# pavel-paulau/query

Hardware: AMD Instinct MI355X
Metric: rows/sec filter+group-by on 100M synthetic JSON docs; achieved HBM GB/s (higher is better)
Workload: dtype int64/f64 tagged scalars (u8 tag + 8 B payload), u32 dictionary codes; 1 GPU; config2: SELECT cat, SUM(price) FROM default WHERE price > 50 GROUP BY cat @ 100000000 rows, K_cat=1000, columns resident in HBM; rows_per_gpu=100000000, groups=1000, rows_selected=49401294, agg_mode=2, spec_kernel=1

## Files before the change

### query_amd/csrc/n1k_kernels.hip

```cpp
#include <hip/hip_runtime.h>
#include "n1k_device.h"
#include "n1k_tables.h"
#include "n1k_scatter.h"
#include "n1k_kernels.h"
#include <algorithm>
#include <vector>

namespace n1k {


template <int R>
N1K_DEV void load_operand(const Program& P, const Operand& o, const uint64_t (&row)[R], const bool (&valid)[R],
                          uint32_t (&tag)[R], uint64_t (&pay)[R]) {
    if (o.is_const) {
#pragma unroll
        for (int j = 0; j < R; j++) {
            tag[j] = o.ctag;
            pay[j] = o.cpayload;
        }
        return;
    }
    const DevCol& c = P.cols[o.col];
    if (c.kind == COLK_DICT32) {
        const uint32_t* codes = c.codes;
// ... 1185 lines not shown
                    unpackable = 1;
                    pass[j] = false;
                }
                key[j] = mix64(key[j] ^ canon) + k;
            }
        }
        uint64_t pos[R];
        uint32_t dest[R];
#pragma unroll
        for (int j = 0; j < R; j++) {
            dest[j] = (uint32_t)(((key[j] >> 32) * (uint64_t)A.nparts) >> 32);
            pos[j] = 0;
            for (uint32_t d = 0; d < A.nparts; d++) {
                unsigned long long m = __ballot(pass[j] && dest[j] == d);
                if (m == 0ull) continue;
                int leader = __ffsll((long long)m) - 1;
                uint32_t base = 0;
                if ((int)lane == leader) base = atomicAdd(&s_cnt[d], (uint32_t)__popcll(m));
                base = __shfl(base, leader, 64);
                if (pass[j] && dest[j] == d) pos[j] = base + (uint32_t)__popcll(m & ((1ull << lane) - 1ull));
            }
        }
        __syncthreads();
        for (uint32_t d = tid; d < A.nparts; d += BLOCK) {
            uint32_t n = s_cnt[d];
            s_base[d] = n ? atomicAdd(&A.counts[(size_t)d * (A.count_stride ? A.count_stride : 1u)], (unsigned long long)n) : 0ull;
        }
        __syncthreads();
#pragma unroll
        for (int j = 0; j < R; j++) {
            if (!pass[j]) continue;
            uint64_t r = s_base[dest[j]] + pos[j];
            if (r >= (A.per_dest ? (uint64_t)A.dest_cap[dest[j]] : A.capacity)) {
                if (!(atomicOr(A.err_flags, (uint32_t)ERR_TABLE_FULL) & ERR_TABLE_FULL) && A.region_bytes)
                    for (uint32_t q = 0; q < A.nparts; q++)
                        atomicOr(&A.counts[(size_t)q * A.count_stride + 1], 1ull);
                pass[j] = false;
            }
            pos[j] = A.region_bytes ? r : (uint64_t)dest[j] * A.capacity + r;
        }
        __syncthreads();
        for (uint32_t d = tid; d < A.nparts; d += BLOCK) s_cnt[d] = 0;
        uint64_t roff[R];
#pragma unroll
        for (int j = 0; j < R; j++) roff[j] = A.hdr_bytes;
        for (uint32_t c = 0; c < A.ncopy; c++) {
            Operand o{};
            o.is_const = 0;
            o.col = c;
            uint32_t vt[R];
            uint64_t vp[R];
            load_operand<R>(P, o, row, pass, vt, vp);
#pragma unroll
            for (int j = 0; j < R; j++) {
                if (!pass[j]) continue;
                if (A.per_dest) {
                    char* const reg = (char*)A.counts + (size_t)dest[j] * A.region_bytes;
                    const uint64_t capd = A.dest_cap[dest[j]];
                    if (P.cols[c].kind == COLK_DICT32) {
                        ((uint32_t*)(reg + roff[j]))[pos[j]] = (uint32_t)vp[j];
                        roff[j] = part_region_next(roff[j], capd, 4);
                    } else {
                        ((uint64_t*)(reg + roff[j]))[pos[j]] = vp[j];
                        roff[j] = part_region_next(roff[j], capd, 8);
                        ((uint8_t*)(reg + roff[j]))[pos[j]] = (uint8_t)vt[j];
                        roff[j] = part_region_next(roff[j], capd, 1);
                    }
                    continue;
                }
                const size_t shift = (size_t)dest[j] * A.region_bytes;
                if (P.cols[c].kind == COLK_DICT32) {
                    ((uint32_t*)((char*)A.out_codes[c] + shift))[pos[j]] = (uint32_t)vp[j];
                } else {
                    ((uint8_t*)((char*)A.out_tags[c] + shift))[pos[j]] = (uint8_t)vt[j];
                    ((uint64_t*)((char*)A.out_payload[c] + shift))[pos[j]] = vp[j];
                }
            }
        }
    }
    if (unsupported) atomicOr(A.err_flags, (uint32_t)ERR_UNSUPPORTED_VALUE);
    if (unpackable) atomicOr(A.err_flags, (uint32_t)ERR_UNPACKABLE_KEY);
}

enum { RED_ADD_U64, RED_ADD_F64, RED_OR, RED_MIN_I64, RED_MAX_I64, RED_MIN_U64, RED_MAX_U64 };

template <int OP>
N1K_DEV uint64_t reduce_over_y(uint64_t (*red)[64], uint64_t v) {
    const uint32_t tx = threadIdx.x, ty = threadIdx.y;
    red[ty][tx] = v;
    __syncthreads();
    for (uint32_t off = 8; off > 0; off >>= 1) {
        if (ty < off) {
            uint64_t a = red[ty][tx], b = red[ty + off][tx], r;
            if (OP == RED_ADD_U64) r = a + b;
            else if (OP == RED_ADD_F64) r = f64_bits(as_f64(a) + as_f64(b));
            else if (OP == RED_OR) r = a | b;
            else if (OP == RED_MIN_I64) r = (int64_t)a < (int64_t)b ? a : b;
            else if (OP == RED_MAX_I64) r = (int64_t)a > (int64_t)b ? a : b;
            else if (OP == RED_MIN_U64) r = a < b ? a : b;
            else r = a > b ? a : b;
            red[ty][tx] = r;
        }
        __syncthreads();
    }
    uint64_t out = red[0][tx];
    __syncthreads();
    return out;
}

__global__ __launch_bounds__(1024) void merge_slabs_kernel(const Program P, const FastArgs F, const GlobalTable G,
                                                          uint32_t nblocks_total, unsigned long long* ngroups) {
    __shared__ uint64_t red[16][64];
    const uint32_t S = F.lds_slots;
    const uint32_t s = blockIdx.x * 64 + threadIdx.x;
    const bool in_range = s < S;
    if (blockIdx.x == 0 && blockIdx.y == 0 && threadIdx.y == 0) {
        unsigned long long c = 0;
        for (uint32_t b = threadIdx.x; b < nblocks_total; b += 64) c += F.block_selected[b];
        for (int off = 32; off > 0; off >>= 1) c += __shfl_down(c, off, 64);
        if (threadIdx.x == 0 && c) atomicAdd(F.rows_selected, c);
    }
    const uint32_t Y = 16 * gridDim.y, y = blockIdx.y * 16 + threadIdx.y;
    const size_t slab_words = (size_t)P.lds_words * S * Y;
    const uint32_t nblocks = (in_range && y < nblocks_total) ? (nblocks_total - y + Y - 1) / Y : 0;
    const uint64_t* base = F.slabs + (size_t)y * P.lds_words * S + (in_range ? s : 0);
    uint64_t touched = 0;
#pragma unroll 8
    for (uint32_t b = 0; b < nblocks; b++) touched |= base[b * slab_words] ^ kEmptyKey;
    touched = reduce_over_y<RED_OR>(red, touched);
    const bool leader = threadIdx.y == 0 && in_range && touched != 0;
    long long g = -1;
    if (leader) g = global_find_or_insert(G, fast_slot_key(F, s), F.err_flags, ngroups);
    uint64_t* grow = g >= 0 ? &G.acc[(size_t)g * P.glob_words] : nullptr;
    for (uint32_t a = 0; a < P.naggs; a++) {
        const AggSpec& ag = P.aggs[a];
        if (ag.distinct) continue;
        const uint64_t* l = base + (size_t)ag.lds_off * S;
        unsigned long long* w = grow ? (unsigned long long*)(grow + ag.glob_off) : nullptr;
        switch (ag.kind) {
            case AGG_COUNT:
            case AGG_COUNTN: {
                unsigned long long c = 0;
#pragma unroll 8
                for (uint32_t b = 0; b < nblocks; b++) c += l[b * slab_words];
                c = reduce_over_y<RED_ADD_U64>(red, c);
                if (w && c) atomicAdd(&w[0], c);
                break;
            }
            case AGG_SUM:
            case AGG_AVG: {
                unsigned long long lo = 0, hi = 0, fl = 0, n = 0;
                double fs = 0.0;
                const bool avg = ag.kind == AGG_AVG;
#pragma unroll 4
                for (uint32_t b = 0; b < nblocks; b++) {
                    const uint64_t* lb = l + b * slab_words;
                    int64_t x = (int64_t)lb[0];
                    double f = as_f64(lb[(size_t)S]);
                    fl |= lb[2 * (size_t)S];
                    lo += (unsigned long long)(uint32_t)x;
                    hi += (unsigned long long)(x >> 32);
                    fs += f;
                    if (avg) n += lb[3 * (size_t)S];
                }
                lo = reduce_over_y<RED_ADD_U64>(red, lo);
                hi = reduce_over_y<RED_ADD_U64>(red, hi);
                fs = as_f64(reduce_over_y<RED_ADD_F64>(red, f64_bits(fs)));
                fl = reduce_over_y<RED_OR>(red, fl);
                if (avg) n = reduce_over_y<RED_ADD_U64>(red, n);
                if (!w || !fl) break;
                if (fl & (SF_NONNEG_INT | SF_NEG_INT)) { atomicAdd(&w[0], lo); atomicAdd(&w[1], hi); }
                if (fl & SF_FLOAT) atomicAdd((double*)&w[2], fs);
                atomicOr(&w[3], fl);
                if (avg) atomicAdd(&w[4], n);
                break;
            }
            default: {
                const bool mn = ag.kind == AGG_MIN;
                unsigned long long fl = 0;
                long long iv = mn ? INT64_MAX : INT64_MIN;
                unsigned long long fv = mn ? ~0ull : 0ull, sv = mn ? ~0ull : 0ull;
#pragma unroll 4
                for (uint32_t b = 0; b < nblocks; b++) {
                    const uint64_t* lb = l + b * slab_words;
                    fl |= lb[0];
                    long long x = (long long)lb[(size_t)S];
                    unsigned long long yv = lb[2 * (size_t)S], z = lb[3 * (size_t)S];
                    iv = mn ? (x < iv ? x : iv) : (x > iv ? x : iv);
                    fv = mn ? (yv < fv ? yv : fv) : (yv > fv ? yv : fv);
                    sv = mn ? (z < sv ? z : sv) : (z > sv ? z : sv);
                }
                fl = reduce_over_y<RED_OR>(red, fl);
                if (mn) {
                    iv = (long long)reduce_over_y<RED_MIN_I64>(red, (uint64_t)iv);
                    fv = reduce_over_y<RED_MIN_U64>(red, fv);
                    sv = reduce_over_y<RED_MIN_U64>(red, sv);
                } else {
                    iv = (long long)reduce_over_y<RED_MAX_I64>(red, (uint64_t)iv);
                    fv = reduce_over_y<RED_MAX_U64>(red, fv);
                    sv = reduce_over_y<RED_MAX_U64>(red, sv);
                }
                if (!w || !fl) break;
                atomicOr(&w[0], fl);
                if (fl & MM_INT) { if (mn) atomicMin((long long*)&w[1], iv); else atomicMax((long long*)&w[1], iv); }
                if (fl & MM_FLOAT) { if (mn) atomicMin(&w[2], fv); else atomicMax(&w[2], fv); }
                if (fl & MM_STRING) { if (mn) atomicMin(&w[3], sv); else atomicMax(&w[3], sv); }
                break;
            }
        }
    }
}

__global__ void export_partials_kernel(const Program P, const GlobalTable G, uint32_t nparts, uint64_t cap,
                                       uint64_t* out, uint64_t region_words, uint32_t* err_flags) {
    uint64_t s = (uint64_t)blockIdx.x * blockDim.x + threadIdx.x;
    if (s == 0 && P.wide_count && *P.wide_count)
        for (uint32_t r = 0; r < nparts; r++) atomicOr((unsigned long long*)&out[(size_t)r * region_words + 1], 2ull);
    const uint64_t key = s < G.capacity ? G.keys[s] : kEmptyKey;
    const bool used = key != kEmptyKey;
    const uint32_t d = used ? (uint32_t)(((mix64(key) >> 32) * (uint64_t)nparts) >> 32) : 0xFFFFFFFFu;
    unsigned long long pos = 0;
    unsigned long long todo = __ballot(used);
    const uint32_t lane = threadIdx.x & 63;
    while (todo) {
        const int leader = __ffsll((long long)todo) - 1;
        const uint32_t dl = __shfl(d, leader, 64);
        const unsigned long long same = __ballot(used && d == dl);
        unsigned long long base = 0;
        if ((int)lane == leader) base = atomicAdd((unsigned long long*)&out[(size_t)dl * region_words], (unsigned long long)__popcll(same));
        base = __shfl(base, leader, 64);
        if (used && d == dl) pos = base + (unsigned long long)__popcll(same & ((1ull << lane) - 1ull));
        todo &= ~same;
    }
    if (!used) return;
    uint64_t* region = out + (size_t)d * region_words;
    if (pos >= cap) {
        if (!(atomicOr(err_flags, (uint32_t)ERR_TABLE_FULL) & ERR_TABLE_FULL))
            for (uint32_t r = 0; r < nparts; r++) atomicOr((unsigned long long*)&out[(size_t)r * region_words + 1], 1ull);
        return;
    }
    region[2 + pos] = key;
    uint64_t* acc = region + 2 + cap + pos * P.glob_words;
    for (uint32_t w = 0; w < P.glob_words; w++) acc[w] = G.acc[(size_t)s * P.glob_words + w];
}

N1K_DEV void merge_partial_record(const Program& P, const GlobalTable& G, uint64_t key, const uint64_t* l, uint32_t* err_flags,
                                  bool& fresh, bool unique_keys) {
    long long g = global_find_or_insert_quiet(G, key, err_flags, fresh);
    if (g < 0) return;
    if (fresh && unique_keys) {
        uint64_t* w = &G.acc[(size_t)g * P.glob_words];
        for (uint32_t i = 0; i < P.glob_words; i++) w[i] = l[i];
        return;
    }
    for (uint32_t a = 0; a < P.naggs; a++) {
        const AggSpec& ag = P.aggs[a];
        const uint64_t* p = l + ag.glob_off;
        unsigned long long* w = (unsigned long long*)&G.acc[(size_t)g * P.glob_words + ag.glob_off];
        if (ag.distinct) {
            atomicOr(err_flags, (uint32_t)ERR_UNSUPPORTED_VALUE);
            continue;
        }
        switch (ag.kind) {
            case AGG_COUNT:
            case AGG_COUNTN:
                if (p[0]) atomicAdd(&w[0], (unsigned long long)p[0]);
                break;
            case AGG_SUM:
            case AGG_AVG:
                if (!p[3]) break;
                atomicAdd(&w[0], (unsigned long long)p[0]);
                atomicAdd(&w[1], (unsigned long long)p[1]);
                if (p[3] & SF_FLOAT) atomicAdd((double*)&w[2], as_f64(p[2]));
                atomicOr(&w[3], (unsigned long long)p[3]);
                if (ag.kind == AGG_AVG) atomicAdd(&w[4], (unsigned long long)p[4]);
                break;
            default: {
                if (!p[0]) break;
                bool mn = ag.kind == AGG_MIN;
                atomicOr(&w[0], (unsigned long long)p[0]);
                if (p[0] & MM_INT) { if (mn) atomicMin((long long*)&w[1], (long long)p[1]); else atomicMax((long long*)&w[1], (long long)p[1]); }
                if (p[0] & MM_FLOAT) { if (mn) atomicMin(&w[2], (unsigned long long)p[2]); else atomicMax(&w[2], (unsigned long long)p[2]); }
                if (p[0] & MM_STRING) { if (mn) atomicMin(&w[3], (unsigned long long)p[3]); else atomicMax(&w[3], (unsigned long long)p[3]); }
                break;
            }
        }
    }
}

N1K_DEV void raise_verdict(uint64_t verdict, uint32_t* err_flags) {
    uint32_t f = 0;
    if (verdict & VD_OVERFLOW) f |= ERR_EXCHANGE_OVERFLOW;
// ... 155 lines not shown
            else which = (fl & MM_OTHER) ? 4 : ((fl & MM_STRING) ? 3 : (has_num ? 2 : (has_bool ? 1 : 0)));
            if (which == 1) {
                tag = mn ? ((fl & MM_FALSE) ? T_FALSE : T_TRUE) : ((fl & MM_TRUE) ? T_TRUE : T_FALSE);
            } else if (which == 2) {
                bool hi = fl & MM_INT, hf = fl & MM_FLOAT;
                double f = f64_unsortable(w[2]);
                int64_t iv = (int64_t)w[1];
                bool pick_int = hi;
                if (hi && hf) {
                    int c = collate_f64((double)iv, f);
                    pick_int = mn ? c <= 0 : c >= 0;
                }
                if (pick_int) { tag = T_INT; p = (uint64_t)iv; }
                else { tag = T_FLOAT; p = f64_bits(f); }
            } else if (which == 3) {
                tag = T_STRING;
                p = w[3] & 0xFFFFFFFFull;
            } else if (which == 4) {
                atomicOr(err_flags, (uint32_t)ERR_UNSUPPORTED_VALUE);
            }
            pt.ext_tag = tag;
            pt.ext_payload = p;
            put_value(fin, tag, p);
            break;
        }
    }
    *part = pt;
}

constexpr uint32_t kFinalizeChunkMax = 16384;
__global__ __launch_bounds__(256) void finalize_kernel(const Program P, const GlobalTable G, OutValue* out_keys, OutValue* out_aggs,
                                                       OutPartial* out_parts, uint64_t* out_rep, unsigned long long* out_count,
                                                       uint64_t max_out, uint32_t* err_flags, uint32_t chunk) {
    __shared__ uint32_t wave_cnt[4];
    __shared__ unsigned long long chunk_base;
    const uint32_t tid = threadIdx.x, lane = tid & 63, wave = tid >> 6;
    const uint64_t lo = (uint64_t)blockIdx.x * chunk;
    const uint64_t hi = lo + chunk < G.capacity ? lo + chunk : G.capacity;
    uint32_t mine = 0;
    for (uint64_t s = lo + tid; s < hi; s += 256) mine += G.keys[s] != kEmptyKey ? 1u : 0u;
    for (int off = 32; off > 0; off >>= 1) mine += __shfl_down(mine, off, 64);
    if (lane == 0) wave_cnt[wave] = mine;
    __syncthreads();
    if (tid == 0) {
        const uint32_t total = wave_cnt[0] + wave_cnt[1] + wave_cnt[2] + wave_cnt[3];
        chunk_base = total ? atomicAdd(out_count, (unsigned long long)total) : 0ull;
    }
    __syncthreads();
    unsigned long long next = chunk_base;
    for (uint64_t s0 = lo; s0 < hi; s0 += 256) {
        const uint64_t s = s0 + tid;
        const uint64_t key = s < hi ? G.keys[s] : kEmptyKey;
        const bool used = key != kEmptyKey;
        const unsigned long long m = __ballot(used);
        __syncthreads();
        if (lane == 0) wave_cnt[wave] = (uint32_t)__popcll(m);
        __syncthreads();
        uint32_t before = 0;
        for (uint32_t w = 0; w < wave; w++) before += wave_cnt[w];
        const uint32_t step_total = wave_cnt[0] + wave_cnt[1] + wave_cnt[2] + wave_cnt[3];
        const unsigned long long idx = next + before + (uint32_t)__popcll(m & ((1ull << lane) - 1ull));
        next += step_total;
        if (!used || idx >= max_out) continue;
        for (uint32_t k = 0; k < P.nkeys; k++) {
            const KeySpec& ks = P.keys[k];
            uint64_t field = ks.bits >= 64 ? key : ((key >> ks.shift) & ((1ull << ks.bits) - 1ull));
            uint32_t tag;
            uint64_t p;
            unpack_key_field(P, ks.mode, field, tag, p);
            put_value(&out_keys[idx * P.nkeys + k], tag, p);
        }
        const uint64_t* g = &G.acc[(size_t)s * P.glob_words];
        for (uint32_t a = 0; a < P.naggs; a++)
            finalize_agg(P, P.aggs[a], g, &out_aggs[idx * P.naggs + a], &out_parts[idx * P.naggs + a], err_flags);
        if (out_rep) out_rep[idx] = P.emit_packed_key ? key : (G.rep_row ? G.rep_row[s] : ~0ull);
    }
}

constexpr uint32_t kFinalizeSmallMax = 8192;
__global__ __launch_bounds__(1024) void finalize_small_kernel(const Program P, const GlobalTable G, OutValue* out_keys, OutValue* out_aggs,
                                                             OutPartial* out_parts, uint64_t* out_rep, unsigned long long* counters,
                                                             unsigned long long* host_counters, uint64_t max_out, uint32_t* err_flags,
                                                             uint32_t clear) {
    __shared__ uint32_t wave_cnt[16];
    const uint32_t tid = threadIdx.x, lane = tid & 63, wave = tid >> 6;
    unsigned long long next = 0;
    for (uint64_t s0 = 0; s0 < G.capacity; s0 += 1024) {
        const uint64_t s = s0 + tid;
        const uint64_t key = s < G.capacity ? G.keys[s] : kEmptyKey;
        const bool used = key != kEmptyKey;
        const unsigned long long m = __ballot(used);
        __syncthreads();
        if (lane == 0) wave_cnt[wave] = (uint32_t)__popcll(m);
        __syncthreads();
        uint32_t before = 0, step_total = 0;
        for (uint32_t w = 0; w < 16; w++) {
            before += w < wave ? wave_cnt[w] : 0u;
            step_total += wave_cnt[w];
        }
        const unsigned long long idx = next + before + (uint32_t)__popcll(m & ((1ull << lane) - 1ull));
        next += step_total;
        if (!used) continue;
        uint64_t* g = &G.acc[(size_t)s * P.glob_words];
        if (idx < max_out) {
            for (uint32_t k = 0; k < P.nkeys; k++) {
                const KeySpec& ks = P.keys[k];
                uint64_t field = ks.bits >= 64 ? key : ((key >> ks.shift) & ((1ull << ks.bits) - 1ull));
                uint32_t tag;
                uint64_t p;
                unpack_key_field(P, ks.mode, field, tag, p);
                put_value(&out_keys[idx * P.nkeys + k], tag, p);
            }
            for (uint32_t a = 0; a < P.naggs; a++)
                finalize_agg(P, P.aggs[a], g, &out_aggs[idx * P.naggs + a], &out_parts[idx * P.naggs + a], err_flags);
            if (out_rep) out_rep[idx] = P.emit_packed_key ? key : (G.rep_row ? G.rep_row[s] : ~0ull);
        }
        if (clear) {
            G.keys[s] = kEmptyKey;
            if (G.rep_row) G.rep_row[s] = ~0ull;
            glob_row_init(P, g);
        }
    }
    __syncthreads();
    if (tid == 0) counters[2] = next;
    __syncthreads();
    if (tid < kCounters) {
        host_counters[tid] = __hip_atomic_load(&counters[tid], __ATOMIC_RELAXED, __HIP_MEMORY_SCOPE_AGENT);
        if (clear) counters[tid] = 0;
    }
}

hipError_t launch_finalize_small(const Program& P, const GlobalTable& G, OutValue* out_keys, OutValue* out_aggs, OutPartial* out_parts,
                                 uint64_t* out_rep, unsigned long long* counters, unsigned long long* host_counters, uint64_t max_out,
                                 uint32_t* err_flags, bool clear, hipStream_t st) {
    if (G.capacity > kFinalizeSmallMax) return hipErrorInvalidValue;
    hipLaunchKernelGGL(finalize_small_kernel, dim3(1), dim3(1024), 0, st, P, G, out_keys, out_aggs, out_parts, out_rep, counters,
                       host_counters, max_out, err_flags, clear ? 1u : 0u);
    return hipGetLastError();
}

N1K_DEV uint64_t order_image(const Program& P, uint64_t tag, uint64_t p, bool desc);
__global__ void finalize_region_kernel(const Program P, const uint64_t* region, uint64_t cap, uint64_t count, OutValue* out_keys,
                                       OutValue* out_aggs, OutPartial* out_parts, uint64_t* out_rep, uint32_t* err_flags,
                                       const uint32_t* cand, OutValue* ord, uint32_t ord_is_key, uint32_t ord_index, uint64_t* images,
                                       uint32_t desc) {
    const uint64_t j = (uint64_t)blockIdx.x * blockDim.x + threadIdx.x;
    if (j >= count) return;
    const uint64_t i = cand ? (uint64_t)cand[j] : j;
    const uint64_t key = region[2 + i];
    const uint64_t* g = region + 2 + cap + i * P.glob_words;
    if (ord || images) {
        OutValue v, term;
        OutPartial part;
        term.tag = T_MISSING;
        term.payload = 0;
        for (uint32_t a = 0; a < P.naggs; a++) {
            finalize_agg(P, P.aggs[a], g, &v, &part, err_flags);
            if (!ord_is_key && a == ord_index) term = v;
        }
        if (ord_is_key) {
            const KeySpec& ks = P.keys[ord_index];
            uint64_t field = ks.bits >= 64 ? key : ((key >> ks.shift) & ((1ull << ks.bits) - 1ull));
            uint32_t tag;
            uint64_t p;
            unpack_key_field(P, ks.mode, field, tag, p);
            put_value(&term, tag, p);
        }
        if (images) images[i] = order_image(P, term.tag, term.payload, desc != 0);
        else ord[i] = term;
        return;
    }
    for (uint32_t k = 0; k < P.nkeys; k++) {
        const KeySpec& ks = P.keys[k];
        uint64_t field = ks.bits >= 64 ? key : ((key >> ks.shift) & ((1ull << ks.bits) - 1ull));
        uint32_t tag;
        uint64_t p;
        unpack_key_field(P, ks.mode, field, tag, p);
        put_value(&out_keys[j * P.nkeys + k], tag, p);
    }
    for (uint32_t a = 0; a < P.naggs; a++)
        finalize_agg(P, P.aggs[a], g, &out_aggs[j * P.naggs + a], &out_parts[j * P.naggs + a], err_flags);
    if (out_rep) out_rep[j] = ~0ull;
}

template <int R, int BLOCK>
__global__ __launch_bounds__(BLOCK) void project_records_kernel(const Program P, const ProjectArgs A) {
    __shared__ uint32_t wave_cnt[BLOCK / 64];
    __shared__ unsigned long long tile_base;
    __shared__ uint32_t s_hist[256];
    const uint32_t tid = threadIdx.x;
    for (uint32_t i = tid; i < 256; i += BLOCK) s_hist[i] = 0;
    __syncthreads();
    uint32_t unsupported = 0, unpackable = 0;
    const uint64_t tile_rows = (uint64_t)BLOCK * R;
    const uint64_t ntiles = (A.nrows + tile_rows - 1) / tile_rows;
    for (uint64_t tile = blockIdx.x; tile < ntiles; tile += gridDim.x) {
        uint64_t row[R];
// ... 750 lines not shown
        } else {
            tag = T_STRING;
            pay = a.k_cat;
        }
        if (a.price_tags) a.price_tags[j] = tag;
        if (a.price_payload) a.price_payload[j] = pay;
    }
    uint64_t urange = a.total_rows / 10;
    if (urange == 0) urange = 1;
    if (a.user_tags) a.user_tags[j] = T_INT;
    if (a.user_payload) a.user_payload[j] = splitmix64(base + 3) % urange;
    if (a.region_tags) a.region_tags[j] = T_INT;
    if (a.region_payload) a.region_payload[j] = splitmix64(base + 4) % 64ull;
}


hipError_t launch_init_table(const Program& P, const GlobalTable& G, uint64_t first, uint64_t count,
                             unsigned long long* counters, hipStream_t st) {
    if (count == 0) return hipSuccess;
    uint32_t blocks = (uint32_t)((count + 255) / 256);
    hipLaunchKernelGGL(init_table_kernel, dim3(blocks), dim3(256), 0, st, P, G, first, count, counters);
    return hipGetLastError();
}

hipError_t launch_rehash(const Program& P, const GlobalTable& oldt, const GlobalTable& newt, uint32_t* err_flags,
                         unsigned long long* ngroups_scratch, hipStream_t st) {
    uint32_t blocks = (uint32_t)((oldt.capacity + 255) / 256);
    hipLaunchKernelGGL(rehash_kernel, dim3(blocks), dim3(256), 0, st, P, oldt, newt, err_flags, ngroups_scratch);
    return hipGetLastError();
}

template <int R, int BLOCK>
static hipError_t launch_scan_variant(const Program& P, const ScanArgs& A, const GlobalTable& G, unsigned long long* ngroups,
                                      uint32_t grid, bool direct, size_t shmem, hipStream_t st) {
    if (direct) {
        auto k = scan_group_kernel<R, BLOCK, true>;
        if (shmem > 48 * 1024) (void)hipFuncSetAttribute((const void*)k, hipFuncAttributeMaxDynamicSharedMemorySize, (int)shmem);
        hipLaunchKernelGGL(k, dim3(grid), dim3(BLOCK), shmem, st, P, A, G, ngroups);
    } else {
        auto k = scan_group_kernel<R, BLOCK, false>;
        if (shmem > 48 * 1024) (void)hipFuncSetAttribute((const void*)k, hipFuncAttributeMaxDynamicSharedMemorySize, (int)shmem);
        hipLaunchKernelGGL(k, dim3(grid), dim3(BLOCK), shmem, st, P, A, G, ngroups);
    }
    return hipGetLastError();
}

hipError_t launch_scan_group(const Program& P, const ScanArgs& A, const GlobalTable& G, unsigned long long* ngroups,
                             uint32_t grid, uint32_t block, uint32_t rows_per_lane, bool direct, hipStream_t st) {
    size_t shmem = (size_t)A.lds_slots * P.lds_words * 8 + (size_t)A.dcache_slots * A.dcache_aggs * 8;
    if (block == 256) return launch_scan_variant<4, 256>(P, A, G, ngroups, grid, direct, shmem, st);
    if (block == 512) return launch_scan_variant<4, 512>(P, A, G, ngroups, grid, direct, shmem, st);
    if (rows_per_lane == 2) return launch_scan_variant<2, 1024>(P, A, G, ngroups, grid, direct, shmem, st);
    return launch_scan_variant<4, 1024>(P, A, G, ngroups, grid, direct, shmem, st);
}

template <int R, int BLOCK>
static hipError_t launch_fast_variant(const Program& P, const FastArgs& F, const GlobalTable& G, unsigned long long* ngroups,
                                      uint32_t grid, size_t shmem, hipStream_t st) {
    auto k = scan_fast_kernel<R, BLOCK>;
    if (shmem > 48 * 1024) (void)hipFuncSetAttribute((const void*)k, hipFuncAttributeMaxDynamicSharedMemorySize, (int)shmem);
    hipLaunchKernelGGL(k, dim3(grid), dim3(BLOCK), shmem, st, P, F, G, ngroups);
    return hipGetLastError();
}

hipError_t launch_scan_fast(const Program& P, const FastArgs& F, const GlobalTable& G, unsigned long long* ngroups,
                            uint32_t grid, uint32_t block, uint32_t rows_per_lane, hipStream_t st) {
    size_t shmem = (size_t)F.lds_slots * P.lds_words * 8;
    for (uint32_t t = 0; t < F.nterms; t++)
        if (term_is_table_bit(F.terms[t].op) && F.terms[t].like_n <= kLikeLdsBytes) {
            shmem += kLikeLdsBytes;
            break;
        }
    if (block == 512) {
        if (rows_per_lane == 2) return launch_fast_variant<2, 512>(P, F, G, ngroups, grid, shmem, st);
        return launch_fast_variant<4, 512>(P, F, G, ngroups, grid, shmem, st);
    }
    if (rows_per_lane == 2) return launch_fast_variant<2, 1024>(P, F, G, ngroups, grid, shmem, st);
    return launch_fast_variant<4, 1024>(P, F, G, ngroups, grid, shmem, st);
}

hipError_t launch_merge_slabs(const Program& P, const FastArgs& F, const GlobalTable& G, uint32_t nblocks,
                              unsigned long long* ngroups, hipStream_t st, uint32_t ychunks_opt) {
    uint32_t blocks = (F.lds_slots + 63) / 64;
    uint32_t ychunks = nblocks >= 512 ? 4 : (nblocks >= 128 ? 2 : 1);
    while (ychunks < 16 && blocks * ychunks < 256 && nblocks >= 32 * ychunks) ychunks *= 2;
    if (ychunks_opt) ychunks = ychunks_opt;
    hipLaunchKernelGGL(merge_slabs_kernel, dim3(blocks, ychunks), dim3(64, 16), 0, st, P, F, G, nblocks, ngroups);
    return hipGetLastError();
}

__global__ void add_counter_kernel(unsigned long long* p, unsigned long long v) { *p += v; }

hipError_t launch_add_counter(unsigned long long* p, unsigned long long v, hipStream_t st) {
    hipLaunchKernelGGL(add_counter_kernel, dim3(1), dim3(1), 0, st, p, v);
    return hipGetLastError();
}

hipError_t launch_finalize_region(const Program& P, const uint64_t* region, uint64_t cap, uint64_t count, OutValue* out_keys,
                                  OutValue* out_aggs, OutPartial* out_parts, uint64_t* out_rep, uint32_t* err_flags, hipStream_t st,
                                  const uint32_t* cand, OutValue* ord, bool ord_is_key, uint32_t ord_index, uint64_t* images, bool desc) {
    if (!count) return hipSuccess;
    hipLaunchKernelGGL(finalize_region_kernel, dim3((uint32_t)((count + 255) / 256)), dim3(256), 0, st, P, region, cap, count,
                       out_keys, out_aggs, out_parts, out_rep, err_flags, cand, ord, ord_is_key ? 1u : 0u, ord_index, images, desc ? 1u : 0u);
    return hipGetLastError();
}

hipError_t launch_probe_keys(const Program& P, uint64_t nrows, const GlobalTable& G, uint32_t* err_flags, unsigned long long* ngroups,
                             uint32_t grid, hipStream_t st) {
    hipLaunchKernelGGL((probe_keys_kernel<4, 256>), dim3(grid), dim3(256), 0, st, P, nrows, G, err_flags, ngroups);
    return hipGetLastError();
}

hipError_t launch_project_records(const Program& P, const ProjectArgs& A, uint32_t grid, hipStream_t st) {
    hipLaunchKernelGGL((project_records_kernel<4, 512>), dim3(grid), dim3(512), 0, st, P, A);
    return hipGetLastError();
}

hipError_t launch_agg_bins(const Program& P, const BinAggArgs& A, const GlobalTable& G, unsigned long long* ngroups, uint32_t grid,
                           hipStream_t st) {
    auto k = agg_bins_kernel<512>;
    size_t shmem = (size_t)A.lds_slots * P.lds_words * 8;
    if (shmem > 48 * 1024) (void)hipFuncSetAttribute((const void*)k, hipFuncAttributeMaxDynamicSharedMemorySize, (int)shmem);
    hipLaunchKernelGGL(k, dim3(grid), dim3(512), shmem, st, P, A, G, ngroups);
    return hipGetLastError();
}

size_t topk_state_bytes() { return sizeof(TopkState); }

uint64_t topk_cand_entries(uint64_t n) { return n + (uint64_t)kTopkSegs * (n / kTopkSegs + 320); }
bool topk_can_sample(uint64_t n, uint64_t keep) { return n >= 4ull * kTopkSample && n < (1ull << 32) && keep * 2 * kTopkSample / n + 16 <= kTopkSample / 4; }

hipError_t launch_topk_select(const Program& P, const OutValue* vals, uint32_t stride, uint32_t index, uint64_t n, bool desc,
                              uint64_t keep, uint64_t* images, void* state, uint32_t* cand, hipStream_t st, bool sampled,
                              bool images_done) {
    TopkState* S = (TopkState*)state;
    (void)hipMemsetAsync(S, 0, sizeof(TopkState), st);
    const uint32_t blocks = (uint32_t)((n + 255) / 256);
    if (!images_done)
        hipLaunchKernelGGL(topk_images_kernel, dim3(blocks), dim3(256), 0, st, P, vals, stride, index, n, desc ? 1u : 0u, images, S, keep);
    else
        hipLaunchKernelGGL(topk_state_kernel, dim3(1), dim3(1), 0, st, S, keep);
    if (sampled) {
        const uint32_t rank = (uint32_t)(keep * 2 * kTopkSample / n) + 16;
        auto k = topk_sample_kernel;
        (void)hipFuncSetAttribute((const void*)k, hipFuncAttributeMaxDynamicSharedMemorySize, (int)(kTopkSample * 8));
        hipLaunchKernelGGL(k, dim3(1), dim3(1024), kTopkSample * 8, st, images, n, rank, S);
        const uint64_t seg_cap = n / kTopkSegs + 320;
        uint32_t* seg_lists = cand + n;
        hipLaunchKernelGGL(topk_gather_seg_kernel, dim3(blocks), dim3(256), 0, st, images, n, S, seg_lists, seg_cap);
        auto kr = topk_refine_kernel;
        (void)hipFuncSetAttribute((const void*)kr, hipFuncAttributeMaxDynamicSharedMemorySize, (int)(kTopkSample * 8));
        hipLaunchKernelGGL(kr, dim3(1), dim3(1024), kTopkSample * 8, st, images, S, seg_lists, seg_cap, cand, keep);
        return hipGetLastError();
    }
    const uint32_t hb = (uint32_t)std::min<uint64_t>(blocks, 1024);
    for (uint32_t pass = 0; pass < 8; pass++) {
        hipLaunchKernelGGL(topk_hist_kernel, dim3(hb), dim3(256), 0, st, images, n, pass, S);
        hipLaunchKernelGGL(topk_pick_kernel, dim3(1), dim3(64), 0, st, pass, S);
    }
    hipLaunchKernelGGL(topk_gather_kernel, dim3(blocks), dim3(256), 0, st, images, n, S, cand);
    return hipGetLastError();
}

size_t topk_ncand_offset() { return offsetof(TopkState, ncand); }

hipError_t launch_topk_compact(const uint32_t* cand, uint64_t ncand, uint32_t nk, uint32_t na, const OutValue* keys,
                               const OutValue* aggs, const OutPartial* parts, const uint64_t* rep, OutValue* okeys, OutValue* oaggs,
                               OutPartial* oparts, uint64_t* orep, hipStream_t st) {
// ... 227 lines not shown
```

Before: 331.3 billion rows/s.

## Batch slab loads and single-sync reductions in merge and finalize-small kernels

Restructures merge_slabs_kernel so each thread issues loads for four slabs at once and prefetches the next aggregate's words while reducing the current one. The per-value log-step reduction with a __syncthreads per step is replaced by one shared-memory store of all accumulator words, followed by a single-thread-row tree reduction. The finalize-small kernel now compacts occupied slots with one wave-level prefix scan instead of a looped ballot with barriers per 1024 slots. The ychunks heuristic is retuned for the new per-thread slab batching. This targets latency and barrier overhead in the post-scan merge/finalize phase, at the cost of more registers and LDS.

New measurement: 332.3 billion rows/s, median of 3. Within noise of the previous version (+0.3%).

```diff
diff --git a/query_amd/csrc/n1k_kernels.hip b/query_amd/csrc/n1k_kernels.hip
--- a/query_amd/csrc/n1k_kernels.hip
+++ b/query_amd/csrc/n1k_kernels.hip
@@ -1291,132 +1291,234 @@
     if (unpackable) atomicOr(A.err_flags, (uint32_t)ERR_UNPACKABLE_KEY);
 }
 
-enum { RED_ADD_U64, RED_ADD_F64, RED_OR, RED_MIN_I64, RED_MAX_I64, RED_MIN_U64, RED_MAX_U64 };
+enum { RED_ADD_U64, RED_ADD_F64, RED_OR, RED_MIN_I64, RED_MIN_U64 };
+
+constexpr int kMergeSlabs = 4;
+constexpr int kMergeWords = 5;
+
+N1K_DEV uint32_t merge_agg_words(const AggSpec& ag) {
+    return (ag.kind == AGG_COUNT || ag.kind == AGG_COUNTN) ? 1u
+           : (ag.kind == AGG_SUM ? kLdsWordsSum : (ag.kind == AGG_AVG ? kLdsWordsAvg : kWordsMinMax));
+}
+
+N1K_DEV void merge_issue(const uint64_t* slabs, const uint32_t (&sb)[kMergeSlabs], size_t slab_words, uint32_t word0, uint32_t nw,
+                         size_t S, uint64_t (&raw)[kMergeSlabs][4]) {
+#pragma unroll
+    for (int j = 0; j < kMergeSlabs; j++) {
+#pragma unroll
+        for (uint32_t i = 0; i < 3; i++) raw[j][i] = slabs[sb[j] * slab_words + (size_t)(word0 + (i < nw ? i : 0u)) * S];
+    }
+    if (nw > 3) {
+#pragma unroll
+        for (int j = 0; j < kMergeSlabs; j++) raw[j][3] = slabs[sb[j] * slab_words + (size_t)(word0 + 3u) * S];
+    } else {
+#pragma unroll
+        for (int j = 0; j < kMergeSlabs; j++) raw[j][3] = 0;
+    }
+}
+
+N1K_DEV void merge_acc_init(uint32_t kind, uint64_t (&acc)[kMergeWords]) {
+#pragma unroll
+    for (int i = 0; i < kMergeWords; i++) acc[i] = 0;
+    if (kind == AGG_MIN) { acc[1] = (uint64_t)INT64_MAX; acc[2] = ~0ull; acc[3] = ~0ull; }
+    if (kind == AGG_MAX) acc[1] = (uint64_t)INT64_MIN;
+}
+
+N1K_DEV void merge_fold(uint32_t kind, uint64_t (&acc)[kMergeWords], const uint64_t (&w)[kMergeSlabs][4], const bool (&ok)[kMergeSlabs]) {
+    switch (kind) {
+        case AGG_COUNT:
+        case AGG_COUNTN:
+#pragma unroll
+            for (int j = 0; j < kMergeSlabs; j++) acc[0] += ok[j] ? w[j][0] : 0ull;
+            break;
+        case AGG_SUM:
+        case AGG_AVG:
+#pragma unroll
+            for (int j = 0; j < kMergeSlabs; j++) {
+                const int64_t x = ok[j] ? (int64_t)w[j][0] : 0;
+                const double f = ok[j] ? as_f64(w[j][1]) : 0.0;
+                acc[0] += (unsigned long long)(uint32_t)x;
+                acc[1] += (unsigned long long)(x >> 32);
+                acc[2] = f64_bits(as_f64(acc[2]) + f);
+                acc[3] |= ok[j] ? w[j][2] : 0ull;
+                if (kind == AGG_AVG) acc[4] += ok[j] ? w[j][3] : 0ull;
+            }
+            break;
+        default: {
+            const bool mn = kind == AGG_MIN;
+#pragma unroll
+            for (int j = 0; j < kMergeSlabs; j++) {
+                const long long x = ok[j] ? (long long)w[j][1] : (mn ? INT64_MAX : INT64_MIN);
+                const unsigned long long yv = ok[j] ? w[j][2] : (mn ? ~0ull : 0ull), z = ok[j] ? w[j][3] : (mn ? ~0ull : 0ull);
+                const long long iv = (long long)acc[1];
+                acc[0] |= ok[j] ? w[j][0] : 0ull;
+                acc[1] = (uint64_t)(mn ? (x < iv ? x : iv) : (x > iv ? x : iv));
+                acc[2] = mn ? (yv < acc[2] ? yv : acc[2]) : (yv > acc[2] ? yv : acc[2]);
+                acc[3] = mn ? (z < acc[3] ? z : acc[3]) : (z > acc[3] ? z : acc[3]);
+            }
+            break;
+        }
+    }
+}
 
 template <int OP>
-N1K_DEV uint64_t reduce_over_y(uint64_t (*red)[64], uint64_t v) {
-    const uint32_t tx = threadIdx.x, ty = threadIdx.y;
-    red[ty][tx] = v;
-    __syncthreads();
-    for (uint32_t off = 8; off > 0; off >>= 1) {
-        if (ty < off) {
-            uint64_t a = red[ty][tx], b = red[ty + off][tx], r;
-            if (OP == RED_ADD_U64) r = a + b;
-            else if (OP == RED_ADD_F64) r = f64_bits(as_f64(a) + as_f64(b));
-            else if (OP == RED_OR) r = a | b;
-            else if (OP == RED_MIN_I64) r = (int64_t)a < (int64_t)b ? a : b;
-            else if (OP == RED_MAX_I64) r = (int64_t)a > (int64_t)b ? a : b;
-            else if (OP == RED_MIN_U64) r = a < b ? a : b;
-            else r = a > b ? a : b;
-            red[ty][tx] = r;
-        }
-        __syncthreads();
-    }
-    uint64_t out = red[0][tx];
-    __syncthreads();
-    return out;
+N1K_DEV uint64_t reduce_op(uint64_t a, uint64_t b, bool mx) {
+    if (OP == RED_ADD_U64) return a + b;
+    if (OP == RED_ADD_F64) return f64_bits(as_f64(a) + as_f64(b));
+    if (OP == RED_OR) return a | b;
+    if (OP == RED_MIN_I64) return ((int64_t)a < (int64_t)b) != mx ? a : b;
+    return (a < b) != mx ? a : b;
+}
+
+template <int OP>
+N1K_DEV uint64_t reduce_rows(const uint64_t (*plane)[64], uint32_t& tx, bool mx = false) {
+    uint64_t r[8];
+#pragma unroll
+    for (int h = 0; h < 2; h++) {
+        uint64_t lo[4], hi[4];
+#pragma unroll
+        for (int i = 0; i < 4; i++) { lo[i] = plane[h * 4 + i][tx]; hi[i] = plane[h * 4 + i + 8][tx]; }
+#pragma unroll
+        for (int i = 0; i < 4; i++) r[h * 4 + i] = reduce_op<OP>(lo[i], hi[i], mx);
+        asm volatile("" : "+v"(tx) : "v"(r[h * 4 + 3]));
+    }
+#pragma unroll
+    for (int off = 4; off > 0; off >>= 1) {
+#pragma unroll
+        for (int i = 0; i < off; i++) r[i] = reduce_op<OP>(r[i], r[i + off], mx);
+    }
+    asm volatile("" : "+v"(tx) : "v"(r[0]));
+    return r[0];
 }
 
 __global__ __launch_bounds__(1024) void merge_slabs_kernel(const Program P, const FastArgs F, const GlobalTable G,
                                                           uint32_t nblocks_total, unsigned long long* ngroups) {
-    __shared__ uint64_t red[16][64];
+    __shared__ uint64_t red[kMergeWords + 1][16][64];
     const uint32_t S = F.lds_slots;
-    const uint32_t s = blockIdx.x * 64 + threadIdx.x;
+    const uint32_t tx = threadIdx.x, ty = threadIdx.y;
+    const uint32_t s = blockIdx.x * 64 + tx;
     const bool in_range = s < S;
-    if (blockIdx.x == 0 && blockIdx.y == 0 && threadIdx.y == 0) {
+    const uint32_t Y = 16 * gridDim.y, y = blockIdx.y * 16 + ty;
+    const uint32_t rounds = (nblocks_total + kMergeSlabs * Y - 1) / (kMergeSlabs * Y);
+    const size_t slab_words = (size_t)P.lds_words * S;
+    const uint32_t home = y < nblocks_total ? y : 0u;
+    const uint64_t* const slabs = F.slabs + (in_range ? s : 0u);
+    uint32_t sb[kMergeSlabs];
+    bool ok[kMergeSlabs];
+#pragma unroll
+    for (int j = 0; j < kMergeSlabs; j++) {
+        const uint32_t b = y + (uint32_t)j * Y;
+        ok[j] = in_range && b < nblocks_total;
+        sb[j] = ok[j] ? b : home;
+    }
+    uint32_t a0 = 0;
+    while (a0 < P.naggs && P.aggs[a0].distinct) a0++;
+    uint64_t kw[kMergeSlabs], raw[kMergeSlabs][4];
+#pragma unroll
+    for (int j = 0; j < kMergeSlabs; j++) kw[j] = slabs[sb[j] * slab_words];
+    if (a0 < P.naggs) merge_issue(slabs, sb, slab_words, P.aggs[a0].lds_off, merge_agg_words(P.aggs[a0]), S, raw);
+    if (blockIdx.x == 0 && blockIdx.y == 0 && ty == 0) {
         unsigned long long c = 0;
-        for (uint32_t b = threadIdx.x; b < nblocks_total; b += 64) c += F.block_selected[b];
-        for (int off = 32; off > 0; off >>= 1) c += __shfl_down(c, off, 64);
-        if (threadIdx.x == 0 && c) atomicAdd(F.rows_selected, c);
-    }
-    const uint32_t Y = 16 * gridDim.y, y = blockIdx.y * 16 + threadIdx.y;
-    const size_t slab_words = (size_t)P.lds_words * S * Y;
-    const uint32_t nblocks = (in_range && y < nblocks_total) ? (nblocks_total - y + Y - 1) / Y : 0;
-    const uint64_t* base = F.slabs + (size_t)y * P.lds_words * S + (in_range ? s : 0);
+        for (uint32_t b = tx; b < nblocks_total; b += 64) c += F.block_selected[b];
+        for (int o = 32; o > 0; o >>= 1) c += __shfl_down(c, o, 64);
+        if (tx == 0 && c) atomicAdd(F.rows_selected, c);
+    }
     uint64_t touched = 0;
-#pragma unroll 8
-    for (uint32_t b = 0; b < nblocks; b++) touched |= base[b * slab_words] ^ kEmptyKey;
-    touched = reduce_over_y<RED_OR>(red, touched);
-    const bool leader = threadIdx.y == 0 && in_range && touched != 0;
-    long long g = -1;
-    if (leader) g = global_find_or_insert(G, fast_slot_key(F, s), F.err_flags, ngroups);
-    uint64_t* grow = g >= 0 ? &G.acc[(size_t)g * P.glob_words] : nullptr;
-    for (uint32_t a = 0; a < P.naggs; a++) {
+#pragma unroll
+    for (int j = 0; j < kMergeSlabs; j++) touched |= ok[j] ? (kw[j] ^ kEmptyKey) : 0ull;
+    for (uint32_t r = 1; r < rounds; r++) {
+        uint64_t k2[kMergeSlabs];
+        bool ok2[kMergeSlabs];
+#pragma unroll
+        for (int j = 0; j < kMergeSlabs; j++) {
+            const uint32_t b = y + (r * kMergeSlabs + (uint32_t)j) * Y;
+            ok2[j] = in_range && b < nblocks_total;
+            k2[j] = slabs[(size_t)(ok2[j] ? b : home) * slab_words];
+        }
+#pragma unroll
+        for (int j = 0; j < kMergeSlabs; j++) touched |= ok2[j] ? (k2[j] ^ kEmptyKey) : 0ull;
+    }
+    red[kMergeWords][ty][tx] = touched;
+    unsigned long long* grow = nullptr;
+    auto open_row = [&](uint32_t& cx) {
+        const uint64_t t = reduce_rows<RED_OR>(red[kMergeWords], cx);
+        if (in_range && t != 0) {
+            const long long g = global_find_or_insert(G, fast_slot_key(F, s), F.err_flags, ngroups);
+            if (g >= 0) grow = (unsigned long long*)&G.acc[(size_t)g * P.glob_words];
+        }
+    };
+    bool first = true, loaded = true;
+    for (uint32_t a = a0; a < P.naggs; a++) {
         const AggSpec& ag = P.aggs[a];
         if (ag.distinct) continue;
-        const uint64_t* l = base + (size_t)ag.lds_off * S;
-        unsigned long long* w = grow ? (unsigned long long*)(grow + ag.glob_off) : nullptr;
-        switch (ag.kind) {
-            case AGG_COUNT:
-            case AGG_COUNTN: {
-                unsigned long long c = 0;
-#pragma unroll 8
-                for (uint32_t b = 0; b < nblocks; b++) c += l[b * slab_words];
-                c = reduce_over_y<RED_ADD_U64>(red, c);
-                if (w && c) atomicAdd(&w[0], c);
-                break;
-            }
-            case AGG_SUM:
-            case AGG_AVG: {
-                unsigned long long lo = 0, hi = 0, fl = 0, n = 0;
-                double fs = 0.0;
-                const bool avg = ag.kind == AGG_AVG;
-#pragma unroll 4
-                for (uint32_t b = 0; b < nblocks; b++) {
-                    const uint64_t* lb = l + b * slab_words;
-                    int64_t x = (int64_t)lb[0];
-                    double f = as_f64(lb[(size_t)S]);
-                    fl |= lb[2 * (size_t)S];
-                    lo += (unsigned long long)(uint32_t)x;
-                    hi += (unsigned long long)(x >> 32);
-                    fs += f;
-                    if (avg) n += lb[3 * (size_t)S];
-                }
-                lo = reduce_over_y<RED_ADD_U64>(red, lo);
-                hi = reduce_over_y<RED_ADD_U64>(red, hi);
-                fs = as_f64(reduce_over_y<RED_ADD_F64>(red, f64_bits(fs)));
-                fl = reduce_over_y<RED_OR>(red, fl);
-                if (avg) n = reduce_over_y<RED_ADD_U64>(red, n);
-                if (!w || !fl) break;
-                if (fl & (SF_NONNEG_INT | SF_NEG_INT)) { atomicAdd(&w[0], lo); atomicAdd(&w[1], hi); }
-                if (fl & SF_FLOAT) atomicAdd((double*)&w[2], fs);
-                atomicOr(&w[3], fl);
-                if (avg) atomicAdd(&w[4], n);
-                break;
-            }
-            default: {
-                const bool mn = ag.kind == AGG_MIN;
-                unsigned long long fl = 0;
-                long long iv = mn ? INT64_MAX : INT64_MIN;
-                unsigned long long fv = mn ? ~0ull : 0ull, sv = mn ? ~0ull : 0ull;
-#pragma unroll 4
-                for (uint32_t b = 0; b < nblocks; b++) {
-                    const uint64_t* lb = l + b * slab_words;
-                    fl |= lb[0];
-                    long long x = (long long)lb[(size_t)S];
-                    unsigned long long yv = lb[2 * (size_t)S], z = lb[3 * (size_t)S];
-                    iv = mn ? (x < iv ? x : iv) : (x > iv ? x : iv);
-                    fv = mn ? (yv < fv ? yv : fv) : (yv > fv ? yv : fv);
-                    sv = mn ? (z < sv ? z : sv) : (z > sv ? z : sv);
-                }
-                fl = reduce_over_y<RED_OR>(red, fl);
-                if (mn) {
-                    iv = (long long)reduce_over_y<RED_MIN_I64>(red, (uint64_t)iv);
-                    fv = reduce_over_y<RED_MIN_U64>(red, fv);
-                    sv = reduce_over_y<RED_MIN_U64>(red, sv);
-                } else {
-                    iv = (long long)reduce_over_y<RED_MAX_I64>(red, (uint64_t)iv);
-                    fv = reduce_over_y<RED_MAX_U64>(red, fv);
-                    sv = reduce_over_y<RED_MAX_U64>(red, sv);
-                }
-                if (!w || !fl) break;
-                atomicOr(&w[0], fl);
-                if (fl & MM_INT) { if (mn) atomicMin((long long*)&w[1], iv); else atomicMax((long long*)&w[1], iv); }
-                if (fl & MM_FLOAT) { if (mn) atomicMin(&w[2], fv); else atomicMax(&w[2], fv); }
-                if (fl & MM_STRING) { if (mn) atomicMin(&w[3], sv); else atomicMax(&w[3], sv); }
-                break;
-            }
-        }
+        const uint32_t kind = ag.kind, nw = merge_agg_words(ag);
+        if (!loaded) merge_issue(slabs, sb, slab_words, ag.lds_off, nw, S, raw);
+        uint64_t acc[kMergeWords];
+        merge_acc_init(kind, acc);
+        merge_fold(kind, acc, raw, ok);
+        for (uint32_t r = 1; r < rounds; r++) {
+            uint32_t sb2[kMergeSlabs];
+            bool ok2[kMergeSlabs];
+#pragma unroll
+            for (int j = 0; j < kMergeSlabs; j++) {
+                const uint32_t b = y + (r * kMergeSlabs + (uint32_t)j) * Y;
+                ok2[j] = in_range && b < nblocks_total;
+                sb2[j] = ok2[j] ? b : home;
+            }
+            merge_issue(slabs, sb2, slab_words, ag.lds_off, nw, S, raw);
+            merge_fold(kind, acc, raw, ok2);
+        }
+        loaded = a + 1 < P.naggs && !P.aggs[a + 1].distinct;
+        if (loaded) merge_issue(slabs, sb, slab_words, P.aggs[a + 1].lds_off, merge_agg_words(P.aggs[a + 1]), S, raw);
+        if (!first) __syncthreads();
+#pragma unroll
+        for (int i = 0; i < kMergeWords; i++) red[i][ty][tx] = acc[i];
+        __syncthreads();
+        if (ty == 0) {
+            uint32_t cx = tx;
+            if (first) open_row(cx);
+            unsigned long long* w = grow ? grow + ag.glob_off : nullptr;
+            switch (kind) {
+                case AGG_COUNT:
+                case AGG_COUNTN: {
+                    const unsigned long long c = reduce_rows<RED_ADD_U64>(red[0], cx);
+                    if (w && c) atomicAdd(&w[0], c);
+                    break;
+                }
+                case AGG_SUM:
+                case AGG_AVG: {
+                    const bool avg = kind == AGG_AVG;
+                    const unsigned long long lo = reduce_rows<RED_ADD_U64>(red[0], cx), hi = reduce_rows<RED_ADD_U64>(red[1], cx);
+                    const double fs = as_f64(reduce_rows<RED_ADD_F64>(red[2], cx));
+                    const unsigned long long fl = reduce_rows<RED_OR>(red[3], cx);
+                    const unsigned long long n = avg ? reduce_rows<RED_ADD_U64>(red[4], cx) : 0ull;
+                    if (!w || !fl) break;
+                    if (fl & (SF_NONNEG_INT | SF_NEG_INT)) { atomicAdd(&w[0], lo); atomicAdd(&w[1], hi); }
+                    if (fl & SF_FLOAT) atomicAdd((double*)&w[2], fs);
+                    atomicOr(&w[3], fl);
+                    if (avg) atomicAdd(&w[4], n);
+                    break;
+                }
+                default: {
+                    const bool mn = kind == AGG_MIN;
+                    const unsigned long long fl = reduce_rows<RED_OR>(red[0], cx);
+                    const long long iv = (long long)reduce_rows<RED_MIN_I64>(red[1], cx, !mn);
+                    const unsigned long long fv = reduce_rows<RED_MIN_U64>(red[2], cx, !mn), sv = reduce_rows<RED_MIN_U64>(red[3], cx, !mn);
+                    if (!w || !fl) break;
+                    atomicOr(&w[0], fl);
+                    if (fl & MM_INT) { if (mn) atomicMin((long long*)&w[1], iv); else atomicMax((long long*)&w[1], iv); }
+                    if (fl & MM_FLOAT) { if (mn) atomicMin(&w[2], fv); else atomicMax(&w[2], fv); }
+                    if (fl & MM_STRING) { if (mn) atomicMin(&w[3], sv); else atomicMax(&w[3], sv); }
+                    break;
+                }
+            }
+        }
+        first = false;
+    }
+    if (first) {
+        __syncthreads();
+        uint32_t cx = tx;
+        if (ty == 0) open_row(cx);
     }
 }
 
@@ -1738,27 +1840,47 @@
                                                              OutPartial* out_parts, uint64_t* out_rep, unsigned long long* counters,
                                                              unsigned long long* host_counters, uint64_t max_out, uint32_t* err_flags,
                                                              uint32_t clear) {
-    __shared__ uint32_t wave_cnt[16];
+    constexpr uint32_t kTurns = kFinalizeSmallMax / 1024;
+    __shared__ uint32_t wave_cnt[kTurns * 16];
+    __shared__ uint16_t slot_of[kFinalizeSmallMax];
     const uint32_t tid = threadIdx.x, lane = tid & 63, wave = tid >> 6;
-    unsigned long long next = 0;
-    for (uint64_t s0 = 0; s0 < G.capacity; s0 += 1024) {
-        const uint64_t s = s0 + tid;
-        const uint64_t key = s < G.capacity ? G.keys[s] : kEmptyKey;
-        const bool used = key != kEmptyKey;
-        const unsigned long long m = __ballot(used);
-        __syncthreads();
-        if (lane == 0) wave_cnt[wave] = (uint32_t)__popcll(m);
-        __syncthreads();
-        uint32_t before = 0, step_total = 0;
-        for (uint32_t w = 0; w < 16; w++) {
-            before += w < wave ? wave_cnt[w] : 0u;
-            step_total += wave_cnt[w];
-        }
-        const unsigned long long idx = next + before + (uint32_t)__popcll(m & ((1ull << lane) - 1ull));
-        next += step_total;
-        if (!used) continue;
+    uint64_t tkey[kTurns];
+#pragma unroll
+    for (uint32_t t = 0; t < kTurns; t++) {
+        const uint32_t s = t * 1024 + tid;
+        tkey[t] = G.keys[s < G.capacity ? s : 0];
+    }
+    unsigned long long m[kTurns];
+#pragma unroll
+    for (uint32_t t = 0; t < kTurns; t++) {
+        m[t] = __ballot(t * 1024 + tid < G.capacity && tkey[t] != kEmptyKey);
+        if (lane == 0) wave_cnt[t * 16 + wave] = (uint32_t)__popcll(m[t]);
+    }
+    __syncthreads();
+    const uint32_t c0 = wave_cnt[2 * lane], c1 = wave_cnt[2 * lane + 1];
+    uint32_t inc = c0 + c1;
+#pragma unroll
+    for (int d = 1; d < 64; d <<= 1) {
+        const uint32_t up = __shfl_up(inc, d, 64);
+        if ((int)lane >= d) inc += up;
+    }
+    const unsigned long long next = __shfl(inc, 63, 64);
+    const uint32_t ex0 = inc - c0 - c1, ex1 = ex0 + c0;
+#pragma unroll
+    for (uint32_t t = 0; t < kTurns; t++) {
+        const uint32_t e = t * 16 + wave;
+        const uint32_t a = __shfl(ex0, (int)(e >> 1), 64), b = __shfl(ex1, (int)(e >> 1), 64);
+        if ((m[t] >> lane) & 1ull)
+            slot_of[((e & 1u) ? b : a) + (uint32_t)__popcll(m[t] & ((1ull << lane) - 1ull))] = (uint16_t)(t * 1024 + tid);
+    }
+    __syncthreads();
+    for (uint64_t idx = tid; idx < next; idx += 1024) {
+        const uint64_t s = slot_of[idx];
+        const uint64_t key = G.keys[s];
         uint64_t* g = &G.acc[(size_t)s * P.glob_words];
         if (idx < max_out) {
+            for (uint32_t a = 0; a < P.naggs; a++)
+                finalize_agg(P, P.aggs[a], g, &out_aggs[idx * P.naggs + a], &out_parts[idx * P.naggs + a], err_flags);
             for (uint32_t k = 0; k < P.nkeys; k++) {
                 const KeySpec& ks = P.keys[k];
                 uint64_t field = ks.bits >= 64 ? key : ((key >> ks.shift) & ((1ull << ks.bits) - 1ull));
@@ -1767,8 +1889,6 @@
                 unpack_key_field(P, ks.mode, field, tag, p);
                 put_value(&out_keys[idx * P.nkeys + k], tag, p);
             }
-            for (uint32_t a = 0; a < P.naggs; a++)
-                finalize_agg(P, P.aggs[a], g, &out_aggs[idx * P.naggs + a], &out_parts[idx * P.naggs + a], err_flags);
             if (out_rep) out_rep[idx] = P.emit_packed_key ? key : (G.rep_row ? G.rep_row[s] : ~0ull);
         }
         if (clear) {
@@ -2685,8 +2805,8 @@
 hipError_t launch_merge_slabs(const Program& P, const FastArgs& F, const GlobalTable& G, uint32_t nblocks,
                               unsigned long long* ngroups, hipStream_t st, uint32_t ychunks_opt) {
     uint32_t blocks = (F.lds_slots + 63) / 64;
-    uint32_t ychunks = nblocks >= 512 ? 4 : (nblocks >= 128 ? 2 : 1);
-    while (ychunks < 16 && blocks * ychunks < 256 && nblocks >= 32 * ychunks) ychunks *= 2;
+    uint32_t ychunks = 1;
+    while (ychunks < 16 && nblocks > 16u * kMergeSlabs * ychunks) ychunks *= 2;
     if (ychunks_opt) ychunks = ychunks_opt;
     hipLaunchKernelGGL(merge_slabs_kernel, dim3(blocks, ychunks), dim3(64, 16), 0, st, P, F, G, nblocks, ngroups);
     return hipGetLastError();
```
